# acg-team/ProGraphMSA

Hardware: AMD Instinct MI355X
Metric: DP cell-updates/sec (GCUPS) + wall-clock on 256 seqs × 1000 aa, WAG (higher is better)
Workload: dtype f32

## Files before the change

### prographmsa_amd/csrc/pgm_align_kernels.h

```cpp
#ifndef PGM_ALIGN_KERNELS_H_
#define PGM_ALIGN_KERNELS_H_

#include <hip/hip_runtime.h>
#include <math.h>
#include <type_traits>
#include "pgm_device.h"

#define PGM_NEG_INF (-INFINITY)

__device__ __forceinline__ float pgm_ls_log_add(float x, float add) {
    const float a = 2.44247459618085927548717403238913328776812604856113966238617812902399112761292613763080658235564f;
    const float b = -4.2040783745848554315883301529007786406310628696382695994938550046831869207082846248658671f;
    const float c = -0.72123729809042963774358701619456664388406302428056983119308906451199556380646306f;
    const uint32_t bits = __float_as_uint(x);
    const float e = (float)((int32_t)(bits >> 23) - 126);
    const float d = __uint_as_float(((bits << 9) >> 9) ^ 0x3f000000u);
    float t = __fdiv_rn(b, __fsub_rn(d, c));
    const float u = __fadd_rn(e, a);
    t = __fadd_rn(t, add);
    t = __fadd_rn(t, u);
    return t;
}

__device__ __forceinline__ float pgm_emission_finish(float num, float ay, float bx, float match_init) {
    float q = __fdiv_rn(num, __fmul_rn(ay, bx));
    if (q != q) q = __uint_as_float(0xFFC00000u);
    return pgm_ls_log_add(q, match_init);
}

template <int DMAX, int NODES>
__global__ void __launch_bounds__(NODES) pgm_prep_kernel(const PgmJob *__restrict__ jobs, int *__restrict__ sync, uint32_t sync_ints) {
    extern __shared__ float prep_lds[];
    {
        const uint32_t nthreads = gridDim.x * gridDim.y * gridDim.z * NODES;
        const uint32_t gid = ((blockIdx.z * gridDim.y + blockIdx.y) * gridDim.x + blockIdx.x) * NODES + threadIdx.x;
        for (uint32_t i = gid; i < sync_ints; i += nthreads) sync[i] = 0;
    }
    const PgmJob &J = jobs[blockIdx.x];
    const bool first = blockIdx.y == 0;
    const uint32_t n = first ? J.n1 : J.n2;
    const uint32_t v0 = blockIdx.z * NODES;
    if (v0 >= n) return;
    if (J.tabhdr && J.tabhdr[0] == 0) {
        const uint32_t nc = J.dim + 2u;
        bool any = n - 1u >= v0 && n - 1u < v0 + (uint32_t)NODES;
        for (uint32_t c = 0; c < nc; ++c) {
            const uint32_t r = (uint32_t)J.tabhdr[1u + (first ? 0u : nc) + c];
            any = any || (r != 0u && r - 1u >= v0 && r - 1u < v0 + (uint32_t)NODES);
        }
        if (!any) return;
    }
    const uint32_t D = J.dim, DP = J.dp, ST = D + 1;
    float *Mf = prep_lds;
    float *pif = prep_lds + D * D;
    float *nl = pif + D;
    const uint32_t nn = min((uint32_t)NODES, n - v0);
    {
        const int32_t *pp = first ? J.pp1 : J.pp2;
        const uint32_t *pc = first ? J.pc1 : J.pc2, *pu = first ? J.pu1 : J.pu2;
        const float *pv = first ? J.pv1 : J.pv2;
        PgmTbNode *rec = (first ? J.tb1 : J.tb2) + v0;
        for (uint32_t i = threadIdx.x; i < nn * PGM_TB_PK; i += NODES) {
            const uint32_t node = i / PGM_TB_PK, k = i % PGM_TB_PK;
            const int32_t eb = pp[v0 + node];
            const uint32_t cnt = (uint32_t)(pp[v0 + node + 1] - eb);
            const int32_t e = cnt == 0u ? 0 : eb + (int32_t)min(k, cnt - 1u);
            if (k == 0) rec[node].cnt = cnt;
            rec[node].c[k] = pc[e]; rec[node].v[k] = pv[e]; rec[node].u[k] = pu[e];
        }
    }
    if (!first) for (uint32_t i = threadIdx.x; i < D * D; i += NODES) Mf[i] = (float)J.M[i];
    for (uint32_t i = threadIdx.x; i < D; i += NODES) pif[i] = (float)J.pi[i];
    const double *sites = first ? J.sites1 : J.sites2;
    const uint32_t *smap = first ? J.smap1 : J.smap2;
    float *dst = (first ? J.g1f : J.t2) + (size_t)DP * v0;
    for (uint32_t i = threadIdx.x; i < nn * D; i += NODES) {
        const uint32_t node = v0 + i / D;
        const float g = (float)sites[(size_t)D * (smap ? smap[node] : node) + i % D];
        nl[(i / D) * ST + (i % D)] = g;
        if (first && DP == D) dst[i] = g;
    }
    __syncthreads();
    const uint32_t v = threadIdx.x;
    float g[DMAX];
    float acc = 0.0f;
    if (v < nn) {
#pragma unroll
        for (int k = 0; k < DMAX; ++k) g[k] = ((uint32_t)k < D) ? nl[v * ST + k] : 0.0f;
        float l0 = 0.0f, l1 = 0.0f, l2 = 0.0f, l3 = 0.0f;
        const uint32_t aligned = D / 4u * 4u;
#pragma unroll
        for (int k = 0; k + 3 < DMAX; k += 4) {
            if ((uint32_t)k < aligned) {
                l0 = __fadd_rn(l0, __fmul_rn(g[k], pif[k]));
                l1 = __fadd_rn(l1, __fmul_rn(g[k + 1], pif[k + 1]));
                l2 = __fadd_rn(l2, __fmul_rn(g[k + 2], pif[k + 2]));
                l3 = __fadd_rn(l3, __fmul_rn(g[k + 3], pif[k + 3]));
            }
        }
        acc = __fadd_rn(0.0f, __fadd_rn(__fadd_rn(l0, l2), __fadd_rn(l1, l3)));
#pragma unroll
        for (int k = 0; k < DMAX; ++k)
            if ((uint32_t)k >= aligned && (uint32_t)k < D) acc = __fadd_rn(acc, __fmul_rn(g[k], pif[k]));
        (first ? J.a1 : J.b2)[v0 + v] = acc;
    }
    if (first) {
        if (DP != D && v < nn) {
#pragma unroll
            for (int k = 0; k < DMAX; ++k) if ((uint32_t)k < DP) dst[(size_t)DP * v + k] = g[k];
        }
        return;
    }
    __syncthreads();
    if (v < nn) {
        for (uint32_t k = 0; k < D; ++k) {
            float t = 0.0f;
#pragma unroll
            for (int j = 0; j < DMAX; ++j)
                if ((uint32_t)j < D) t = __fadd_rn(t, __fmul_rn(Mf[j + D * k], g[j]));
            nl[v * ST + k] = t;
        }
    }
    __syncthreads();
    for (uint32_t i = threadIdx.x; i < nn * DP; i += NODES) {
        const uint32_t node = i / DP, k = i % DP;
        dst[i] = k < D ? nl[node * ST + k] : 0.0f;
    }
}

#define PGM_TAB_HDR 136
__global__ void __launch_bounds__(256) pgm_classify_kernel(const PgmJob *__restrict__ jobs) {
    const PgmJob &J = jobs[blockIdx.x];
    if (!J.tabhdr) return;
    const bool first = blockIdx.y == 0;
    const uint32_t n = first ? J.n1 : J.n2, D = J.dim;
    const double *sites = first ? J.sites1 : J.sites2;
    const uint32_t *smap = first ? J.smap1 : J.smap2;
    uint8_t *cls = (uint8_t *)(first ? J.cls1 : J.cls2);
    const float uni = (float)(1.0 / (double)D);
    for (uint32_t v = blockIdx.z * blockDim.x + threadIdx.x; v < n; v += gridDim.z * blockDim.x) {
        const double *col = sites + (size_t)D * (smap ? smap[v] : v);
        uint32_t nz = 0, sym = 0;
        bool same = true;
        float vs = 0.f;
        const float g0 = (float)col[0];
        for (uint32_t k = 0; k < D; ++k) {
            const float g = (float)col[k];
            if (g != 0.0f) { ++nz; sym = k; vs = g; }
            same = same && g == g0;
        }
        uint32_t c = 255u;
        if (nz == 0u) c = D + 1u;
        else if (nz == 1u && vs == 1.0f) c = sym;
        else if (same && g0 == uni) c = D;
        cls[v] = (uint8_t)c;
        if (c == 255u) atomicOr(J.tabhdr, 1);
        else atomicCAS(J.tabhdr + 1 + (first ? 0u : D + 2u) + c, 0, (int)v + 1);
    }
}

__device__ __forceinline__ size_t pgm_cell_index(const PgmJob &J, uint32_t y, uint32_t x) {
    const uint32_t b = y / PGM_ROWS, l = PGM_HALO + (y - b * PGM_ROWS);
    return ((size_t)b * J.tsteps + (x + l)) * 64u + l;
}
__device__ __forceinline__ float4 pgm_load_cell(const PgmJob &J, uint32_t y, uint32_t x) {
    return J.cells[pgm_cell_index(J, y, x)];
}

__device__ __forceinline__ float pgm_dpp_wave_shr1(float src, float lane0_value) {
    return __int_as_float(__builtin_amdgcn_update_dpp(__float_as_int(lane0_value), __float_as_int(src), 0x138, 0xf, 0xf, false));
}

#define PGM_GLOBAL __attribute__((address_space(1)))
typedef float pgm_v4f __attribute__((ext_vector_type(4)));
template <class T> __device__ __forceinline__ T pgm_gld(const T *p) { return *(const PGM_GLOBAL T *)(uintptr_t)p; }
#define PGM_EM_TB 4
template <int DP, int RB>
__global__ void __launch_bounds__(4 * PGM_ROWS) pgm_emission_skew_kernel(const PgmJob *__restrict__ jobs) {
    typedef float pgm_v2f __attribute__((ext_vector_type(2)));
    constexpr int NT = DP / 4;
    constexpr int COLS = 64 + PGM_EM_TB * PGM_BLOCK - PGM_HALO - 1;
    constexpr int STR = DP + 1;
    __shared__ pgm_v2f tp[(COLS + 1) * STR];
    __shared__ float bq[COLS];
    const PgmJob &J = jobs[blockIdx.z];
    const uint32_t tb0 = blockIdx.x * PGM_EM_TB;
    const uint32_t rsh = J.rshift, nvb = J.nb << rsh;
    if (tb0 >= J.nblk || 4u * RB * blockIdx.y >= nvb) return;
    if (J.tabhdr && pgm_gld(J.tabhdr) == 0) return;
    auto row_of = [&](uint32_t v, uint32_t lane_) { return ((((v >> rsh) << 6) + lane_) << rsh) | (v & ((1u << rsh) - 1u)); };
    auto sblock_of = [&](uint32_t v, uint32_t tb_) { return ((((size_t)(v >> rsh) * J.nblk + tb_) << rsh) | (v & ((1u << rsh) - 1u))); };
    const uint32_t t0 = tb0 * PGM_BLOCK;
    const int cbase = (int)t0 - 63;
    if ((DP == 20 || DP == 4) && RB == 1) {
        constexpr int TE = DP + 1;
        float *const tab = (float *)tp;
        static_assert(COLS * TE <= (COLS + 1) * STR * 2, "score table must fit the column staging area");
        static_assert(DP > 20 || TE <= 32, "row classes must fit As");
        __shared__ float As[32];
        const uint32_t fb0 = 4u * blockIdx.y + threadIdx.x / PGM_ROWS;
        const uint32_t fl = threadIdx.x % PGM_ROWS;
        const bool active = fb0 < nvb;
        int sym = DP;
        bool plain = true;
        float a_row = 0.f;
        if (active) {
            const uint32_t y = row_of(fb0, fl);
            const uint32_t yc = (y + 1 < J.n1) ? y : 0u;
            const float4 *src = (const float4 *)(J.g1f + (size_t)DP * yc);
            int nz = 0;
#pragma unroll
            for (int q = 0; q < NT; ++q) {
                const float4 v = src[q];
                const float vv[4] = {v.x, v.y, v.z, v.w};
#pragma unroll
                for (int u = 0; u < 4; ++u)
                    if (vv[u] != 0.0f) { ++nz; sym = 4 * q + u; plain = plain && vv[u] == 1.0f; }
            }
            plain = plain && nz <= 1;
            a_row = J.a1[yc];
        }
        if (threadIdx.x < 32) As[threadIdx.x] = 0.f;
        if (__syncthreads_and(plain ? 1 : 0)) {
            if (active) As[sym] = a_row;
            __syncthreads();
            const float mi = J.sc.match_init;
            constexpr int NE = (COLS * TE + 4 * PGM_ROWS - 1) / (4 * PGM_ROWS);
            float tt[NE], tb2[NE];
#pragma unroll
            for (int e = 0; e < NE; ++e) {
                const int i = (int)threadIdx.x + e * 4 * PGM_ROWS;
                const int ci = i / TE, k = i % TE, c = cbase + ci;
                const bool in = i < COLS * TE && c >= 0 && c <= (int)J.ncol;
                tb2[e] = in ? J.b2[c] : 0.f;
                tt[e] = (in && k < DP) ? J.t2[(size_t)DP * c + k] : 0.f;
            }
#pragma unroll
            for (int e = 0; e < NE; ++e) {
                const int i = (int)threadIdx.x + e * 4 * PGM_ROWS;
                if (i < COLS * TE) tab[i] = pgm_emission_finish(0.0f + tt[e], As[i % TE], tb2[e], mi);
            }
            __syncthreads();
            if (!active) return;
            PGM_GLOBAL pgm_v4f *const Sq = (PGM_GLOBAL pgm_v4f *)(uintptr_t)J.S;
            const int l = PGM_HALO + (int)fl;
#pragma unroll 1
            for (int w = 0; w < PGM_EM_TB; ++w) {
                const uint32_t tb = tb0 + w;
                if (tb >= J.nblk) break;
                float out[PGM_BLOCK];
#pragma unroll
                for (int i = 0; i < PGM_BLOCK; ++i) out[i] = tab[((int)(tb * PGM_BLOCK) + i - l - cbase) * TE + sym];
                PGM_GLOBAL pgm_v4f *dst = Sq + (sblock_of(fb0, tb) * 64u + (uint32_t)l) * (PGM_BLOCK / 4);
#pragma unroll
                for (int q = 0; q < PGM_BLOCK / 4; ++q) dst[q] = pgm_v4f{out[4 * q], out[4 * q + 1], out[4 * q + 2], out[4 * q + 3]};
            }
            return;
        }
    }
    const float4 *t2q = (const float4 *)J.t2;
    float *tpf = (float *)tp;
    for (int i = threadIdx.x; i < (COLS + 1) * NT; i += 4 * PGM_ROWS) {
        const int ci = i / NT, q = i % NT, c = cbase + ci;
        float4 v = make_float4(0.f, 0.f, 0.f, 0.f);
        if (c >= 0 && c <= (int)J.ncol) v = t2q[(size_t)NT * c + q];
        const float vv[4] = {v.x, v.y, v.z, v.w};
#pragma unroll
        for (int u = 0; u < 4; ++u) {
            const int k = 4 * q + u;
            if (ci < COLS) tpf[2 * (ci * STR + k)] = vv[u];
            if (ci > 0) tpf[2 * ((ci - 1) * STR + k) + 1] = vv[u];
        }
    }
    for (int i = threadIdx.x; i < COLS; i += 4 * PGM_ROWS) {
        const int col = cbase + i;
        bq[i] = (col >= 0 && col <= (int)J.ncol) ? J.b2[col] : 0.f;
    }
    __syncthreads();
    const uint32_t b0 = (4u * blockIdx.y + threadIdx.x / PGM_ROWS) * RB;
    const int l = PGM_HALO + (int)(threadIdx.x % PGM_ROWS);
    if (b0 >= nvb) return;
    float gy[RB][DP], ay[RB];
#pragma unroll
    for (int r = 0; r < RB; ++r) {
        const uint32_t y = row_of(b0 + (uint32_t)r, (uint32_t)(l - PGM_HALO));
        const uint32_t yc = (y + 1 < J.n1) ? y : 0u;
        const float4 *src = (const float4 *)(J.g1f + (size_t)DP * yc);
#pragma unroll
        for (int q = 0; q < NT; ++q) {
            const float4 v = src[q];
            gy[r][4 * q] = v.x; gy[r][4 * q + 1] = v.y; gy[r][4 * q + 2] = v.z; gy[r][4 * q + 3] = v.w;
        }
        ay[r] = J.a1[yc];
    }
    const float mi = J.sc.match_init;
    const uint32_t nblk = J.nblk;
    PGM_GLOBAL pgm_v4f *const Sq = (PGM_GLOBAL pgm_v4f *)(uintptr_t)J.S;
#pragma unroll 1
    for (int w = 0; w < PGM_EM_TB; ++w) {
        const uint32_t tb = tb0 + w;
        if (tb >= nblk) break;
        float out[RB][PGM_BLOCK];
#pragma unroll
        for (int i = 0; i < PGM_BLOCK; i += 2) {
            const int ci = (int)(tb * PGM_BLOCK) + i - l - cbase;
            const pgm_v2f *tc = tp + ci * STR;
            pgm_v2f acc[RB];
#pragma unroll
            for (int r = 0; r < RB; ++r) acc[r] = pgm_v2f{0.0f, 0.0f};
#pragma unroll
            for (int k = 0; k < DP; ++k) {
                const pgm_v2f tk = tc[k];
#pragma unroll
                for (int r = 0; r < RB; ++r) {
                    const pgm_v2f g = {gy[r][k], gy[r][k]};
                    acc[r] = acc[r] + g * tk;
                }
            }
#pragma unroll
            for (int r = 0; r < RB; ++r) {
                out[r][i] = pgm_emission_finish(acc[r].x, ay[r], bq[ci], mi);
                out[r][i + 1] = pgm_emission_finish(acc[r].y, ay[r], bq[ci + 1], mi);
            }
        }
#pragma unroll
        for (int r = 0; r < RB; ++r) {
            if (b0 + (uint32_t)r < nvb) {
                PGM_GLOBAL pgm_v4f *dst = Sq + (sblock_of(b0 + (uint32_t)r, tb) * 64u + (uint32_t)l) * (PGM_BLOCK / 4);
// ... 2267 lines not shown
```

### prographmsa_amd/csrc/pgm_capi.hip

```cpp
#include <hip/hip_runtime.h>

#include <algorithm>
#include <cmath>
#include <cstdio>
#include <thread>
#include <atomic>
#include <chrono>
#include <queue>
#include <cstdlib>
#include <cstring>
#include <numeric>
#include <optional>
#include <mutex>
#include <string>
#include <unordered_set>
#include <vector>
#include <sys/mman.h>

#include "pgm_align_kernels.h"
#include "pgm_crit_kernels.h"
#include "pgm_nw_kernels.h"
#include "pgm_csprofile_kernels.h"
#include "pgm_dist_kernels.h"
#include "pgm_merge_kernels.h"
// ... 248 lines not shown
    for (int k = 0; k < pgm_ctx::SC_HOST; ++k) if (ctx->sc_host[k]) pinned_free(ctx->sc_host[k]);
    for (int k = 0; k < 2; ++k) if (ctx->sc_ev[k]) (void)hipEventDestroy(ctx->sc_ev[k]);
    for (int k = 0; k < pgm_ctx::C_SLOTS; ++k)
        if (ctx->cache_ptr[k]) slot_free(k, ctx->cache_ptr[k]);
    if (ctx->stream4) (void)hipStreamDestroy(ctx->stream4);
    if (ctx->stream3) (void)hipStreamDestroy(ctx->stream3);
    if (ctx->stream2) (void)hipStreamDestroy(ctx->stream2);
    if (ctx->stream) (void)hipStreamDestroy(ctx->stream);
    delete ctx;
}

int pgm_ctx_device_info(pgm_ctx *ctx, char *name, size_t name_len, int *cu_count) {
    if (!ctx) return fail(PGM_ERR_INVALID, "null ctx");
    if (name && name_len) snprintf(name, name_len, "%s (%s)", ctx->prop.name, ctx->prop.gcnArchName);
    if (cu_count) *cu_count = ctx->prop.multiProcessorCount;
    return PGM_OK;
}

}

namespace {
static hipError_t cache_take(pgm_ctx *ctx, int slot, size_t bytes, void **out, size_t *got) {
    if (ctx->cache_ptr[slot] && ctx->cache_bytes[slot] >= bytes) {
        *out = ctx->cache_ptr[slot]; *got = ctx->cache_bytes[slot];
        ctx->cache_ptr[slot] = nullptr; ctx->cache_bytes[slot] = 0;
        return hipSuccess;
    }
    if (ctx->cache_ptr[slot]) {
        slot_free(slot, ctx->cache_ptr[slot]);
        ctx->cache_ptr[slot] = nullptr; ctx->cache_bytes[slot] = 0;
    }
    *got = bytes;
    if (slot == pgm_ctx::C_HIN) return pinned_alloc(bytes, out);
    return slot == pgm_ctx::C_HOST ? hipHostMalloc(out, bytes, hipHostMallocDefault) : hipMalloc(out, bytes);
}
static void cache_give(pgm_ctx *ctx, int slot, void *p, size_t bytes) {
    if (!p) return;
    if (ctx && (!ctx->cache_ptr[slot] || ctx->cache_bytes[slot] < bytes)) {
        if (ctx->cache_ptr[slot]) slot_free(slot, ctx->cache_ptr[slot]);
        ctx->cache_ptr[slot] = p; ctx->cache_bytes[slot] = bytes;
    } else {
        slot_free(slot, p);
    }
}

static hipError_t scratch_dev(pgm_ctx *ctx, int slot, size_t bytes, void **out) {
    bytes = std::max<size_t>(bytes, 16);
    if (ctx->sc_dev_bytes[slot] < bytes) {
        if (ctx->sc_dev[slot]) (void)hipFree(ctx->sc_dev[slot]);
        ctx->sc_dev[slot] = nullptr; ctx->sc_dev_bytes[slot] = 0;
        const size_t want = bytes + bytes / 4;
        hipError_t e = hipMalloc(&ctx->sc_dev[slot], want);
        if (e != hipSuccess) return e;
        ctx->sc_dev_bytes[slot] = want;
    }
    *out = ctx->sc_dev[slot];
    return hipSuccess;
}
static hipError_t scratch_host(pgm_ctx *ctx, int slot, size_t bytes, void **out) {
    bytes = std::max<size_t>(bytes, 16);
    if (ctx->sc_host_bytes[slot] < bytes) {
        if (ctx->sc_host[slot]) pinned_free(ctx->sc_host[slot]);
        ctx->sc_host[slot] = nullptr; ctx->sc_host_bytes[slot] = 0;
        const size_t want = bytes + bytes / 4;
        hipError_t e = pinned_alloc(want, &ctx->sc_host[slot]);
        if (e != hipSuccess) return e;
        ctx->sc_host_bytes[slot] = want;
    }
    *out = ctx->sc_host[slot];
    return hipSuccess;
}
static hipError_t scratch_events(pgm_ctx *ctx) {
    for (int k = 0; k < 2; ++k)
        if (!ctx->sc_ev[k]) { hipError_t e = hipEventCreate(&ctx->sc_ev[k]); if (e != hipSuccess) return e; }
    return hipSuccess;
}

static hipError_t resident_alloc(pgm_ctx *ctx, size_t bytes, uint8_t **out) {
    bytes = (bytes + 255) / 256 * 256;
    while (ctx->res_chunk < ctx->res_chunks.size() && ctx->res_off + bytes > ctx->res_chunks[ctx->res_chunk].cap) { ++ctx->res_chunk; ctx->res_off = 0; }
    if (ctx->res_chunk == ctx->res_chunks.size()) {
        pgm_ctx::ResChunk c{nullptr, std::max<size_t>(bytes, (size_t)96 << 20)};
        const hipError_t e = hipMalloc((void **)&c.p, c.cap);
        if (e != hipSuccess) return e;
        ctx->res_chunks.push_back(c); ctx->res_off = 0;
    }
    *out = ctx->res_chunks[ctx->res_chunk].p + ctx->res_off;
    ctx->res_off += bytes;
    return hipSuccess;
}

struct HostImage {
    size_t align;
    std::vector<uint8_t> bytes;
    explicit HostImage(size_t a = 256) : align(a) {}
    size_t put(const void *src, size_t n) {
        const size_t o = bytes.size();
        bytes.resize(o + (n + align - 1) / align * align);
        if (src && n) memcpy(bytes.data() + o, src, n);
        return o;
    }
};

struct Buf { void **p; size_t bytes; const void *src; void *dst; bool zero; };

struct StageCall {
    pgm_ctx *ctx;
    const char *what;
    float *ms;
    hipStream_t s;
    hipError_t e;
    bool alloc_failed = false, queued = false, timed = false;
    StageCall(pgm_ctx *c, const char *w, float *t) : ctx(c), what(w), ms(t), s(c->stream), e(hipSetDevice(c->device)) {}
    bool ok() const { return e == hipSuccess; }
    void alloc(hipError_t r) { e = r; alloc_failed = r != hipSuccess; }
    template <class T> void buf(int slot, size_t bytes, T **p) { if (ok()) alloc(scratch_dev(ctx, slot, bytes, (void **)p)); }
    template <class T> void host(int slot, size_t bytes, T **p) { if (ok()) alloc(scratch_host(ctx, slot, bytes, (void **)p)); }
    template <class T> void resident(size_t bytes, T **p) { if (ok()) alloc(resident_alloc(ctx, bytes, (uint8_t **)p)); }
    void up(void *dst, const void *src, size_t bytes) { if (ok() && bytes) { queued = true; e = hipMemcpyAsync(dst, src, bytes, hipMemcpyHostToDevice, s); } }
    void zero(void *dst, size_t bytes) { if (ok() && bytes) { queued = true; e = hipMemsetAsync(dst, 0, bytes, s); } }
    void down(void *dst, const void *src, size_t bytes) { if (ok() && bytes) { queued = true; e = hipMemcpyAsync(dst, src, bytes, hipMemcpyDeviceToHost, s); } }
    void bufs(int first, int end, std::initializer_list<Buf> list) {
        if (ok() && (size_t)(end - first) < list.size()) e = hipErrorInvalidValue;
        for (const Buf &b : list) { buf(first++, b.bytes, b.p); if (b.src) up(*b.p, b.src, b.bytes); }
    }
    bool begin() {
        if (ok()) e = scratch_events(ctx);
        if (ok()) { queued = true; e = hipEventRecord(ctx->sc_ev[0], s); }
        return ok();
    }
    void end() {
        if (ok()) e = hipGetLastError();
        if (ok()) e = hipEventRecord(ctx->sc_ev[1], s);
        timed = ok();
    }
    int finish() {
        if (queued) { const hipError_t es = hipStreamSynchronize(s); if (ok()) e = es; }
        if (ok() && timed && ms) (void)hipEventElapsedTime(ms, ctx->sc_ev[0], ctx->sc_ev[1]);
        if (ok()) return PGM_OK;
        (void)hipGetLastError();
        return fail(alloc_failed && e == hipErrorOutOfMemory ? PGM_ERR_NOMEM : PGM_ERR_DEVICE, std::string(what) + ": " + hipGetErrorString(e));
    }
};

static hipError_t classify_lean_jobs(pgm_ctx *ctx, pgm_align_batch *b) {
    if (!b->d_tabhdr || b->njobs == 0) return hipSuccess;
    hipError_t e = hipMemsetAsync(b->d_tabhdr, 0, 4 * (size_t)PGM_TAB_HDR * b->njobs, ctx->stream);
    if (e != hipSuccess) return e;
    hipLaunchKernelGGL(pgm_classify_kernel, dim3(b->njobs, 2, (b->maxn + 1023) / 1024), dim3(256), 0, ctx->stream, b->d_jobs);
    return hipGetLastError();
}

#define PGM_STATUS_PENDING 0x7ffffff0
struct PrepTier { uint32_t tier, threads; size_t lds; };
static PrepTier prep_tier(uint32_t maxdim) {
    const uint32_t tier = alphabet_tier(maxdim), threads = tier == 64u ? 64u : 256u;
    return {tier, threads, ((size_t)maxdim * maxdim + maxdim + threads * ((size_t)maxdim + 1)) * sizeof(float)};
}
static hipError_t launch_all(pgm_ctx *ctx, pgm_align_batch *b, bool timed) {
    hipStream_t s = ctx->stream;
    const BatchSchedule &S = b->sched;
    hipError_t e;
    for (uint32_t i = 0; i < b->njobs; ++i) ((PgmJob::Result *)(b->h_out + b->res_off[i]))->status = PGM_STATUS_PENDING;
    if (timed && (e = hipEventRecord(b->ev[0], s)) != hipSuccess) return e;
    const PrepTier T = prep_tier(b->maxdim);
    const dim3 pg(b->njobs, 2, (b->maxn + T.threads - 1) / T.threads);
    if (T.tier == 4) hipLaunchKernelGGL((pgm_prep_kernel<4, 256>), pg, dim3(256), T.lds, s, b->d_jobs, b->d_sync, (uint32_t)b->sync_ints);
    else if (T.tier == 20) hipLaunchKernelGGL((pgm_prep_kernel<20, 256>), pg, dim3(256), T.lds, s, b->d_jobs, b->d_sync, (uint32_t)b->sync_ints);
    else hipLaunchKernelGGL((pgm_prep_kernel<64, 64>), pg, dim3(64), T.lds, s, b->d_jobs, b->d_sync, (uint32_t)b->sync_ints);
    if ((e = hipGetLastError()) != hipSuccess) return e;
    if (timed && (e = hipEventRecord(b->ev[1], s)) != hipSuccess) return e;
    const dim3 eg((b->maxnblk + PGM_EM_TB - 1) / PGM_EM_TB, (b->maxnb + 3) / 4, b->njobs);
    if (T.tier == 4) hipLaunchKernelGGL((pgm_emission_skew_kernel<4, 1>), eg, dim3(4 * PGM_ROWS), 0, s, b->d_jobs);
    else if (T.tier == 20) hipLaunchKernelGGL((pgm_emission_skew_kernel<20, 1>), eg, dim3(4 * PGM_ROWS), 0, s, b->d_jobs);
    else hipLaunchKernelGGL((pgm_emission_skew_kernel<64, 1>), eg, dim3(4 * PGM_ROWS), 0, s, b->d_jobs);
    if ((e = hipGetLastError()) != hipSuccess) return e;
    if (timed && (e = hipEventRecord(b->ev[2], s)) != hipSuccess) return e;
    const uint32_t spin_limit = b->test_spin_limit ? b->test_spin_limit : PGM_SPIN_LIMIT, stall_job = b->test_stall_job, stall_band = b->test_stall_band;
    const bool fork = S.nlean != 0;
    const bool bandk = S.nbands != 0;
    const bool tbk = (S.nitems != 0 || bandk) && (S.ntb + S.ntb_c + S.ntb_b) != 0;
    const bool critk = S.ncrit != 0;
    if ((fork || bandk || critk) && (e = hipEventRecord(b->ev_fork, s)) != hipSuccess) return e;
    if (critk && (e = hipStreamWaitEvent(ctx->stream4, b->ev_fork, 0)) != hipSuccess) return e;
    if (fork && (e = hipStreamWaitEvent(ctx->stream2, b->ev_fork, 0)) != hipSuccess) return e;
    if (bandk && (e = hipStreamWaitEvent(ctx->stream3, b->ev_fork, 0)) != hipSuccess) return e;
    const uint32_t nrest = S.nitems - S.ncrit;
    hipStream_t sc = critk ? s : ctx->stream4, sr = critk ? ctx->stream4 : s;
    auto sweep = [&](hipStream_t st, uint32_t workers, const PgmItem *list, uint32_t n, bool c3, uint32_t ticket_off) {
        if (c3) hipLaunchKernelGGL(pgm_crit_kernel, dim3(workers), dim3(64 * PGM_C3_WAVES), 0, st, b->d_jobs, list, n, b->d_sync, spin_limit, stall_job, stall_band, ticket_off);
        else hipLaunchKernelGGL(pgm_fill_kernel, dim3(workers), dim3(64 * PGM_WAVES), 0, st, b->d_jobs, list, n, b->d_sync, spin_limit, stall_job, stall_band, ticket_off);
    };
    auto tracebacks = [&](hipStream_t st, uint32_t workers, uint32_t first, uint32_t n, uint32_t lq_off, uint32_t sybase) {
        hipLaunchKernelGGL(pgm_tb_kernel, dim3(workers), dim3(64 * PGM_WAVES), 0, st, b->d_jobs, b->d_tblist + first, n, b->d_sync, b->test_spin_limit, lq_off, sybase, 1u);
    };
    if (critk) sweep(sc, S.ncrit_workers, b->d_items, S.ncrit, S.crit_c3, (uint32_t)PGM_SY_CRIT_TICKET);
    if (nrest != 0) sweep(sr, S.nworkers, b->d_items + S.ncrit, nrest, S.rest_c3, 1u);
    if ((e = hipGetLastError()) != hipSuccess) return e;
    if (fork) {
        hipLaunchKernelGGL((pgm_lean_kernel<2>), dim3(S.nlean_workers), dim3(64 * PGM_WAVES), 0, ctx->stream2, b->d_jobs, b->d_lean, S.nlean, b->d_sync, spin_limit);
        if ((e = hipGetLastError()) != hipSuccess) return e;
    }
    const uint32_t njp = (b->njobs + 3u) / 4u * 4u;
    if (bandk) {
        hipLaunchKernelGGL(pgm_band_kernel, dim3(S.nband_workers), dim3(64 * PGM_WAVES), 0, ctx->stream3, b->d_jobs, b->d_bands, S.nbands_narrow, S.nbands, S.nband_workers - S.nwide_workers, b->d_sync, spin_limit, stall_job, stall_band);
        if ((e = hipGetLastError()) != hipSuccess) return e;
        if (tbk && S.ntb_b) tracebacks(ctx->stream3, S.ntb_b_workers, S.ntb + S.ntb_c, S.ntb_b, b->lq_off + njp, 8u);
        if ((e = hipGetLastError()) != hipSuccess) return e;
        if ((e = hipEventRecord(b->ev_join_b, ctx->stream3)) != hipSuccess) return e;
    }
    if (critk) {
        if (tbk && S.ntb_c) tracebacks(sc, S.ncrit_workers, S.ntb, S.ntb_c, b->lq_off + 2 * njp, 16u);
        if ((e = hipGetLastError()) != hipSuccess) return e;
    }
    if (tbk && S.ntb) {
        tracebacks(sr, S.ntb_workers, 0u, S.ntb, b->lq_off, 0u);
        if ((e = hipGetLastError()) != hipSuccess) return e;
    }
    if (critk && (e = hipEventRecord(b->ev_join_c, ctx->stream4)) != hipSuccess) return e;
    if (bandk && (e = hipStreamWaitEvent(s, b->ev_join_b, 0)) != hipSuccess) return e;
    if (critk && (e = hipStreamWaitEvent(s, b->ev_join_c, 0)) != hipSuccess) return e;
    if (fork && ((e = hipEventRecord(b->ev_join, ctx->stream2)) != hipSuccess || (e = hipStreamWaitEvent(s, b->ev_join, 0)) != hipSuccess)) return e;
    if (timed && (e = hipEventRecord(b->ev[3], s)) != hipSuccess) return e;
    if (timed && (e = hipEventRecord(b->ev[4], s)) != hipSuccess) return e;
    return hipSuccess;
}
struct SmallLayout { size_t sync, jobs, order, items, lean, tblist, bands, times, tabhdr, total_bands; bool any_lean; };
static SmallLayout layout_small(pgm_align_batch *b) {
    SmallLayout s;
    const uint32_t njobs = b->njobs;
    s.total_bands = 0; s.any_lean = false;
    for (const PgmJob &J : b->jobs) { s.total_bands += J.nb; s.any_lean = s.any_lean || (J.lean && !J.keep_cells); }
    DevLayout SM;
    s.sync = SM.take(b->sync_ints * sizeof(int)); s.jobs = SM.take(sizeof(PgmJob) * std::max(1u, njobs));
    s.order = SM.take(4 * (size_t)std::max(1u, njobs)); s.items = SM.take(sizeof(PgmItem) * std::max<size_t>(1, s.total_bands));
    s.lean = SM.take(4 * (size_t)std::max(1u, njobs)); s.tblist = SM.take(8 * (size_t)std::max(1u, njobs));
    s.bands = SM.take(sizeof(PgmItem) * std::max<size_t>(1, s.total_bands)); s.times = SM.take(16 * (size_t)std::max(1u, njobs) + 16);
    s.tabhdr = SM.take(s.any_lean ? 4 * (size_t)PGM_TAB_HDR * njobs : 16);
    b->small_bytes = SM.bytes;
    return s;
}

static double now_ms() { return std::chrono::duration<double, std::milli>(std::chrono::steady_clock::now().time_since_epoch()).count(); }

struct BatchAlloc {
    std::atomic<int> state{0};
    hipError_t err = hipSuccess, host_err = hipSuccess;
    uint8_t *h_out_dev = nullptr;
    double ms_dev = 0, ms_host = 0, ms_slot[6] = {0, 0, 0, 0, 0, 0};
};
static void take_batch_buffers(pgm_ctx *ctx, pgm_align_batch *b, SmallLayout sm, BatchAlloc *A) {
    const double ta0 = now_ms();
    hipError_t e2 = hipSetDevice(ctx->device);
    double tprev = ta0;
    for (int k = 0; k < 6 && e2 == hipSuccess; ++k) {
        const BatchBuffer &s = kBatchBuffers[k];
        e2 = cache_take(ctx, s.slot, b->*s.bytes, (void **)&(b->*s.ptr), &b->cap[s.slot]);
        const double t = now_ms(); A->ms_slot[k] = t - tprev; tprev = t;
    }
    if (e2 == hipSuccess) {
        b->d_sync = (int *)(b->d_small + sm.sync);
        b->d_jobs = (PgmJob *)(b->d_small + sm.jobs);
        b->d_order = (uint32_t *)(b->d_small + sm.order);
        b->d_items = (PgmItem *)(b->d_small + sm.items);
        b->d_lean = (uint32_t *)(b->d_small + sm.lean);
        b->d_tblist = (int2 *)(b->d_small + sm.tblist);
        b->d_bands = (PgmItem *)(b->d_small + sm.bands);
        b->d_times = (unsigned long long *)(b->d_small + sm.times);
        b->d_tabhdr = sm.any_lean ? (int *)(b->d_small + sm.tabhdr) : nullptr;
    }
    A->err = e2;
    A->state.store(e2 == hipSuccess ? 1 : -1, std::memory_order_release);
    A->ms_dev = now_ms() - ta0;
    if (e2 == hipSuccess) {
        hipError_t e3 = cache_take(ctx, pgm_ctx::C_HOST, b->out_bytes + 64, (void **)&b->h_out, &b->cap[pgm_ctx::C_HOST]);
        if (e3 == hipSuccess) b->h_flag = (int *)(b->h_out + (b->out_bytes + 15) / 16 * 16);
        if (e3 == hipSuccess) e3 = hipHostGetDevicePointer((void **)&A->h_out_dev, b->h_out, 0);
        A->host_err = e3;
    }
    A->ms_host = now_ms() - ta0 - A->ms_dev;
}

struct CreateGuard {
    pgm_ctx *ctx;
    pgm_align_batch *b;
    std::thread alloc;
    ~CreateGuard() { if (alloc.joinable()) alloc.join(); if (b) pgm_align_batch_destroy(ctx, b); }
    pgm_align_batch *release() { pgm_align_batch *r = b; b = nullptr; return r; }
};

static void bind_job_pointers(pgm_align_batch *b, const std::vector<JobOff> &off, const pgm_site_ref *res1, const pgm_site_ref *res2, uint8_t *h_out_dev) {
    for (uint32_t i = 0; i < b->njobs; ++i) {
        PgmJob &J = b->jobs[i];
        const JobOff &o = off[i];
        uint8_t *in = b->d_in, *w = b->d_work, *ob = b->d_out;
        J.sites1 = site_ref_of(res1, i) ? res1[i].dev_sites : (const double *)(in + o.s1.sites);
        J.sites2 = site_ref_of(res2, i) ? res2[i].dev_sites : (const double *)(in + o.s2.sites);
        J.smap1 = o.s1.has_smap ? (const uint32_t *)(in + o.s1.smap) : nullptr;
        J.smap2 = o.s2.has_smap ? (const uint32_t *)(in + o.s2.smap) : nullptr;
        J.M = (const double *)(in + o.M); J.pi = (const double *)(in + o.pi);
        J.ni1 = (const PgmNode2 *)(in + o.s1.ni); J.ni2 = (const PgmNode2 *)(in + o.s2.ni);
        J.xp1 = (const int32_t *)(in + o.s1.xp); J.xp2 = (const int32_t *)(in + o.s2.xp);
        J.xc1 = (const uint32_t *)(in + o.s1.xc); J.xc2 = (const uint32_t *)(in + o.s2.xc);
        J.xv1 = (const float *)(in + o.s1.xv); J.xv2 = (const float *)(in + o.s2.xv);
        J.fp1 = (const int32_t *)(in + o.s1.fp); J.fe1 = (const uint2 *)(in + o.s1.fe);
        J.ov2 = (const uint2 *)(in + o.s2.ov);
        J.pp1 = (const int32_t *)(in + o.s1.pp); J.pp2 = (const int32_t *)(in + o.s2.pp);
        J.pc1 = (const uint32_t *)(in + o.s1.pc); J.pc2 = (const uint32_t *)(in + o.s2.pc);
        J.pv1 = (const float *)(in + o.s1.pv); J.pv2 = (const float *)(in + o.s2.pv);
        J.pu1 = (const uint32_t *)(in + o.s1.pu); J.pu2 = (const uint32_t *)(in + o.s2.pu);
        J.g1f = (float *)(w + o.g1f); J.a1 = (float *)(w + o.a1);
        J.t2 = (float *)(w + o.t2); J.b2 = (float *)(w + o.aux2);
        J.map1 = (uint32_t *)(ob + o.map1); J.map2 = (uint32_t *)(ob + o.map2);
        J.mark_score = (float *)(w + o.ms); J.mark_prev = (uint32_t *)(w + o.mp);
        J.tb1 = (PgmTbNode *)(w + o.tb1); J.tb2 = (PgmTbNode *)(w + o.tb2);
        J.result = (PgmJob::Result *)(ob + o.res);
        J.hmap1 = (uint32_t *)(h_out_dev + o.map1); J.hmap2 = (uint32_t *)(h_out_dev + o.map2);
        J.hresult = (PgmJob::Result *)(h_out_dev + o.res);
        J.cells = (float4 *)(b->d_cells + o.cells);
        J.codes = (uint32_t *)(w + o.codes);
        J.endcell = (float4 *)(w + o.endcell);
        if (J.lean && !J.keep_cells && b->d_tabhdr) { J.cls1 = w + o.cls; J.cls2 = w + o.cls + J.n1; J.tabhdr = b->d_tabhdr + (size_t)PGM_TAB_HDR * i; }
// ... 394 lines not shown
```

Measured before the change: 81.92.

## Restructure prep kernel: 256 threads, split k across wavefronts, batched loads

The prep kernel now always runs 256 threads and lets the 20/64-letter tiers handle 64 nodes per block, with wavefronts splitting the M·g matrix-vector product across k ranges. Global loads for the pointer arrays, smap, pi, M, traceback records and site columns are issued up front into registers and staged through LDS before being written, which increases memory-level parallelism. The early-exit check is parallelised across threads with __syncthreads_or. The row pitch DP becomes the compile-time DMAX. This only matches the old behaviour if J.dp always equals the tier size, which is a correctness risk.

After: 81.45. Within noise of the previous version (-0.6%).

```diff
diff --git a/prographmsa_amd/csrc/pgm_align_kernels.h b/prographmsa_amd/csrc/pgm_align_kernels.h
--- a/prographmsa_amd/csrc/pgm_align_kernels.h
+++ b/prographmsa_amd/csrc/pgm_align_kernels.h
@@ -28,12 +28,22 @@
     return pgm_ls_log_add(q, match_init);
 }
 
+#define PGM_GLOBAL __attribute__((address_space(1)))
+typedef float pgm_v4f __attribute__((ext_vector_type(4)));
+template <class T> __device__ __forceinline__ T pgm_gld(const T *p) { return *(const PGM_GLOBAL T *)(uintptr_t)p; }
+template <class T> __device__ __forceinline__ void pgm_gst(T *p, T v) { *(PGM_GLOBAL T *)(uintptr_t)p = v; }
+
+#define PGM_PREP_THREADS 256
+constexpr size_t pgm_prep_lds_floats(size_t dim, size_t nodes) { return 2 * nodes + 1 + dim * dim + dim + nodes * (dim | 1); }
 template <int DMAX, int NODES>
-__global__ void __launch_bounds__(NODES) pgm_prep_kernel(const PgmJob *__restrict__ jobs, int *__restrict__ sync, uint32_t sync_ints) {
+__global__ void __launch_bounds__(PGM_PREP_THREADS) pgm_prep_kernel(const PgmJob *__restrict__ jobs, int *__restrict__ sync, uint32_t sync_ints) {
+    constexpr uint32_t NT = PGM_PREP_THREADS, KQ = NT / NODES, KC = DMAX / KQ;
+    static_assert(NODES % 64 == 0 && KQ * NODES == NT && KC * KQ == DMAX && DMAX + 2 <= (int)NT, "whole wavefronts per part of k");
     extern __shared__ float prep_lds[];
+    const uint32_t tid = threadIdx.x;
     {
-        const uint32_t nthreads = gridDim.x * gridDim.y * gridDim.z * NODES;
-        const uint32_t gid = ((blockIdx.z * gridDim.y + blockIdx.y) * gridDim.x + blockIdx.x) * NODES + threadIdx.x;
+        const uint32_t nthreads = gridDim.x * gridDim.y * gridDim.z * NT;
+        const uint32_t gid = ((blockIdx.z * gridDim.y + blockIdx.y) * gridDim.x + blockIdx.x) * NT + tid;
         for (uint32_t i = gid; i < sync_ints; i += nthreads) sync[i] = 0;
     }
     const PgmJob &J = jobs[blockIdx.x];
@@ -41,53 +51,106 @@
     const uint32_t n = first ? J.n1 : J.n2;
     const uint32_t v0 = blockIdx.z * NODES;
     if (v0 >= n) return;
-    if (J.tabhdr && J.tabhdr[0] == 0) {
-        const uint32_t nc = J.dim + 2u;
-        bool any = n - 1u >= v0 && n - 1u < v0 + (uint32_t)NODES;
-        for (uint32_t c = 0; c < nc; ++c) {
-            const uint32_t r = (uint32_t)J.tabhdr[1u + (first ? 0u : nc) + c];
-            any = any || (r != 0u && r - 1u >= v0 && r - 1u < v0 + (uint32_t)NODES);
-        }
-        if (!any) return;
-    }
-    const uint32_t D = J.dim, DP = J.dp, ST = D + 1;
-    float *Mf = prep_lds;
-    float *pif = prep_lds + D * D;
+    const uint32_t D = J.dim, ST = D | 1u;
+    constexpr uint32_t DP = DMAX;
+    if (J.tabhdr) {
+        const uint32_t nc = D + 2u;
+        const int some_unclassed = pgm_gld(J.tabhdr);
+        const uint32_t r = (uint32_t)pgm_gld(J.tabhdr + 1u + (first ? 0u : nc) + min(tid, nc - 1u));
+        if (some_unclassed == 0) {
+            const bool any = (n - 1u >= v0 && n - 1u < v0 + (uint32_t)NODES)
+                             || (r != 0u && r - 1u >= v0 && r - 1u < v0 + (uint32_t)NODES);
+            if (!__syncthreads_or(any ? 1 : 0)) return;
+        }
+    }
+    int *lp = (int *)prep_lds;
+    uint32_t *ls = (uint32_t *)prep_lds + NODES + 1;
+    float *Mf = prep_lds + 2 * NODES + 1;
+    float *pif = Mf + D * D;
     float *nl = pif + D;
     const uint32_t nn = min((uint32_t)NODES, n - v0);
-    {
-        const int32_t *pp = first ? J.pp1 : J.pp2;
-        const uint32_t *pc = first ? J.pc1 : J.pc2, *pu = first ? J.pu1 : J.pu2;
-        const float *pv = first ? J.pv1 : J.pv2;
-        PgmTbNode *rec = (first ? J.tb1 : J.tb2) + v0;
-        for (uint32_t i = threadIdx.x; i < nn * PGM_TB_PK; i += NODES) {
-            const uint32_t node = i / PGM_TB_PK, k = i % PGM_TB_PK;
-            const int32_t eb = pp[v0 + node];
-            const uint32_t cnt = (uint32_t)(pp[v0 + node + 1] - eb);
-            const int32_t e = cnt == 0u ? 0 : eb + (int32_t)min(k, cnt - 1u);
-            if (k == 0) rec[node].cnt = cnt;
-            rec[node].c[k] = pc[e]; rec[node].v[k] = pv[e]; rec[node].u[k] = pu[e];
-        }
-    }
-    if (!first) for (uint32_t i = threadIdx.x; i < D * D; i += NODES) Mf[i] = (float)J.M[i];
-    for (uint32_t i = threadIdx.x; i < D; i += NODES) pif[i] = (float)J.pi[i];
+    const int32_t *pp = first ? J.pp1 : J.pp2;
+    const uint32_t *pc = first ? J.pc1 : J.pc2, *pu = first ? J.pu1 : J.pu2;
+    const float *pv = first ? J.pv1 : J.pv2;
+    PgmTbNode *rec = (first ? J.tb1 : J.tb2) + v0;
     const double *sites = first ? J.sites1 : J.sites2;
     const uint32_t *smap = first ? J.smap1 : J.smap2;
     float *dst = (first ? J.g1f : J.t2) + (size_t)DP * v0;
-    for (uint32_t i = threadIdx.x; i < nn * D; i += NODES) {
-        const uint32_t node = v0 + i / D;
-        const float g = (float)sites[(size_t)D * (smap ? smap[node] : node) + i % D];
-        nl[(i / D) * ST + (i % D)] = g;
-        if (first && DP == D) dst[i] = g;
+    {
+        constexpr int NPP = (NODES + NT) / NT, NM = (DMAX * DMAX + (int)NT - 1) / (int)NT;
+        int ppv[NPP];
+        double mv[NM];
+#pragma unroll
+        for (int u = 0; u < NPP; ++u) ppv[u] = pgm_gld(pp + v0 + min(tid + NT * u, nn));
+        const uint32_t nd = v0 + min(tid, nn - 1u);
+        const uint32_t sm = smap ? pgm_gld(smap + nd) : nd;
+        const double pd = pgm_gld(J.pi + min(tid, D - 1u));
+        if (!first) {
+#pragma unroll
+            for (int u = 0; u < NM; ++u) mv[u] = pgm_gld(J.M + min(tid + NT * u, D * D - 1u));
+        }
+#pragma unroll
+        for (int u = 0; u < NPP; ++u) if (tid + NT * u <= (uint32_t)NODES) lp[tid + NT * u] = ppv[u];
+        if (tid < (uint32_t)NODES) ls[tid] = sm;
+        if (tid < D) pif[tid] = (float)pd;
+        if (!first) {
+#pragma unroll
+            for (int u = 0; u < NM; ++u) if (tid + NT * u < D * D) Mf[tid + NT * u] = (float)mv[u];
+        }
     }
     __syncthreads();
-    const uint32_t v = threadIdx.x;
+    {
+        constexpr int NR = NODES * PGM_TB_PK / (int)NT, NC = DMAX * NODES / (int)NT;
+        uint32_t rc[NR], ru[NR], rcnt[NR];
+        float rv[NR];
+        double cv[NC];
+#pragma unroll
+        for (int u = 0; u < NR; ++u) {
+            const uint32_t i = tid + NT * u, node = i / PGM_TB_PK, k = i % PGM_TB_PK;
+            const int32_t eb = lp[node];
+            const uint32_t cnt = (uint32_t)(lp[node + 1] - eb);
+            const int32_t e = cnt == 0u ? 0 : eb + (int32_t)min(k, cnt - 1u);
+            rcnt[u] = cnt;
+            rc[u] = pgm_gld(pc + e); rv[u] = pgm_gld(pv + e); ru[u] = pgm_gld(pu + e);
+        }
+        const uint32_t qs = NT / D, rs = NT % D;
+        uint32_t cn = tid / D, ck = tid % D;
+        uint32_t lo[NC];
+#pragma unroll
+        for (int u = 0; u < NC; ++u) {
+            const bool in = cn < nn;
+            lo[u] = in ? cn * ST + ck : 0xffffffffu;
+            cv[u] = pgm_gld(sites + (size_t)D * ls[in ? cn : 0u] + (in ? ck : 0u));
+            cn += qs; ck += rs;
+            if (ck >= D) { ck -= D; ++cn; }
+        }
+#pragma unroll
+        for (int u = 0; u < NR; ++u) {
+            const uint32_t i = tid + NT * u, node = i / PGM_TB_PK, k = i % PGM_TB_PK;
+            if (node < nn) {
+                if (k == 0) pgm_gst(&rec[node].cnt, rcnt[u]);
+                pgm_gst(&rec[node].c[k], rc[u]); pgm_gst(&rec[node].v[k], rv[u]); pgm_gst(&rec[node].u[k], ru[u]);
+            }
+        }
+#pragma unroll
+        for (int u = 0; u < NC; ++u) {
+            if (lo[u] != 0xffffffffu) {
+                const float g = (float)cv[u];
+                nl[lo[u]] = g;
+                if (first && DP == D) pgm_gst(dst + tid + NT * u, g);
+            }
+        }
+    }
+    __syncthreads();
+    const uint32_t v = tid % NODES;
+    const uint32_t kq = KQ == 1 ? 0u : (uint32_t)__builtin_amdgcn_readfirstlane((int)(tid / NODES));
     float g[DMAX];
-    float acc = 0.0f;
     if (v < nn) {
 #pragma unroll
         for (int k = 0; k < DMAX; ++k) g[k] = ((uint32_t)k < D) ? nl[v * ST + k] : 0.0f;
-        float l0 = 0.0f, l1 = 0.0f, l2 = 0.0f, l3 = 0.0f;
+    }
+    if (v < nn && kq == 0u) {
+        float acc, l0 = 0.0f, l1 = 0.0f, l2 = 0.0f, l3 = 0.0f;
         const uint32_t aligned = D / 4u * 4u;
 #pragma unroll
         for (int k = 0; k + 3 < DMAX; k += 4) {
@@ -102,29 +165,26 @@
 #pragma unroll
         for (int k = 0; k < DMAX; ++k)
             if ((uint32_t)k >= aligned && (uint32_t)k < D) acc = __fadd_rn(acc, __fmul_rn(g[k], pif[k]));
-        (first ? J.a1 : J.b2)[v0 + v] = acc;
-    }
-    if (first) {
-        if (DP != D && v < nn) {
-#pragma unroll
-            for (int k = 0; k < DMAX; ++k) if ((uint32_t)k < DP) dst[(size_t)DP * v + k] = g[k];
-        }
-        return;
-    }
-    __syncthreads();
-    if (v < nn) {
-        for (uint32_t k = 0; k < D; ++k) {
-            float t = 0.0f;
-#pragma unroll
-            for (int j = 0; j < DMAX; ++j)
-                if ((uint32_t)j < D) t = __fadd_rn(t, __fmul_rn(Mf[j + D * k], g[j]));
-            nl[v * ST + k] = t;
-        }
-    }
-    __syncthreads();
-    for (uint32_t i = threadIdx.x; i < nn * DP; i += NODES) {
+        pgm_gst((first ? J.a1 : J.b2) + v0 + v, acc);
+    }
+    if (first && DP == D) return;
+    if (!first) {
+        __syncthreads();
+        if (v < nn) {
+            const uint32_t kend = min(D, KC * (kq + 1u));
+            for (uint32_t k = KC * kq; k < kend; ++k) {
+                float t = 0.0f;
+#pragma unroll
+                for (int j = 0; j < DMAX; ++j)
+                    if ((uint32_t)j < D) t = __fadd_rn(t, __fmul_rn(Mf[j + D * k], g[j]));
+                nl[v * ST + k] = t;
+            }
+        }
+        __syncthreads();
+    }
+    for (uint32_t i = tid; i < nn * DP; i += NT) {
         const uint32_t node = i / DP, k = i % DP;
-        dst[i] = k < D ? nl[node * ST + k] : 0.0f;
+        pgm_gst(dst + i, k < D ? nl[node * ST + k] : 0.0f);
     }
 }
 
@@ -171,9 +231,6 @@
     return __int_as_float(__builtin_amdgcn_update_dpp(__float_as_int(lane0_value), __float_as_int(src), 0x138, 0xf, 0xf, false));
 }
 
-#define PGM_GLOBAL __attribute__((address_space(1)))
-typedef float pgm_v4f __attribute__((ext_vector_type(4)));
-template <class T> __device__ __forceinline__ T pgm_gld(const T *p) { return *(const PGM_GLOBAL T *)(uintptr_t)p; }
 #define PGM_EM_TB 4
 template <int DP, int RB>
 __global__ void __launch_bounds__(4 * PGM_ROWS) pgm_emission_skew_kernel(const PgmJob *__restrict__ jobs) {
diff --git a/prographmsa_amd/csrc/pgm_capi.hip b/prographmsa_amd/csrc/pgm_capi.hip
--- a/prographmsa_amd/csrc/pgm_capi.hip
+++ b/prographmsa_amd/csrc/pgm_capi.hip
@@ -424,10 +424,10 @@
 }
 
 #define PGM_STATUS_PENDING 0x7ffffff0
-struct PrepTier { uint32_t tier, threads; size_t lds; };
+struct PrepTier { uint32_t tier, nodes; size_t lds; };
 static PrepTier prep_tier(uint32_t maxdim) {
-    const uint32_t tier = alphabet_tier(maxdim), threads = tier == 64u ? 64u : 256u;
-    return {tier, threads, ((size_t)maxdim * maxdim + maxdim + threads * ((size_t)maxdim + 1)) * sizeof(float)};
+    const uint32_t tier = alphabet_tier(maxdim), nodes = tier == 4u ? 256u : 64u;
+    return {tier, nodes, pgm_prep_lds_floats(maxdim, nodes) * sizeof(float)};
 }
 static hipError_t launch_all(pgm_ctx *ctx, pgm_align_batch *b, bool timed) {
     hipStream_t s = ctx->stream;
@@ -436,10 +436,10 @@
     for (uint32_t i = 0; i < b->njobs; ++i) ((PgmJob::Result *)(b->h_out + b->res_off[i]))->status = PGM_STATUS_PENDING;
     if (timed && (e = hipEventRecord(b->ev[0], s)) != hipSuccess) return e;
     const PrepTier T = prep_tier(b->maxdim);
-    const dim3 pg(b->njobs, 2, (b->maxn + T.threads - 1) / T.threads);
-    if (T.tier == 4) hipLaunchKernelGGL((pgm_prep_kernel<4, 256>), pg, dim3(256), T.lds, s, b->d_jobs, b->d_sync, (uint32_t)b->sync_ints);
-    else if (T.tier == 20) hipLaunchKernelGGL((pgm_prep_kernel<20, 256>), pg, dim3(256), T.lds, s, b->d_jobs, b->d_sync, (uint32_t)b->sync_ints);
-    else hipLaunchKernelGGL((pgm_prep_kernel<64, 64>), pg, dim3(64), T.lds, s, b->d_jobs, b->d_sync, (uint32_t)b->sync_ints);
+    const dim3 pg(b->njobs, 2, (b->maxn + T.nodes - 1) / T.nodes), pb(PGM_PREP_THREADS);
+    if (T.tier == 4) hipLaunchKernelGGL((pgm_prep_kernel<4, 256>), pg, pb, T.lds, s, b->d_jobs, b->d_sync, (uint32_t)b->sync_ints);
+    else if (T.tier == 20) hipLaunchKernelGGL((pgm_prep_kernel<20, 64>), pg, pb, T.lds, s, b->d_jobs, b->d_sync, (uint32_t)b->sync_ints);
+    else hipLaunchKernelGGL((pgm_prep_kernel<64, 64>), pg, pb, T.lds, s, b->d_jobs, b->d_sync, (uint32_t)b->sync_ints);
     if ((e = hipGetLastError()) != hipSuccess) return e;
     if (timed && (e = hipEventRecord(b->ev[1], s)) != hipSuccess) return e;
     const dim3 eg((b->maxnblk + PGM_EM_TB - 1) / PGM_EM_TB, (b->maxnb + 3) / 4, b->njobs);
```
